# duckdb-faiss-ext/duckdb-faiss-ext

Hardware: AMD Instinct MI355X
Metric: queries/sec, FlatL2 d=128 N=10000000 nq=10000 k=10 (higher is better)
Workload: dtype f32 results (bf16 matrix-pipe coarse filter with a proven bound + exact f32 re-scoring of the candidates); 1 GPU; Flat L2 d=128 N=10000000 nq=10000 k=10; queries_per_call=10000, replicas=1, exchange=none

## Files before the change

duckdb-faiss-ext_amd/csrc/collect_launch.h:

```cpp
#pragma once
#include "common.h"

#include <algorithm>
#include <cmath>
#include <cstddef>
#include <cstdint>

namespace mvs {

struct CandStream {
	unsigned long long *entries = nullptr;
	float *values = nullptr;
	unsigned long long *count = nullptr;
	int64_t cap = 0;
};
struct FailList {
	int *count = nullptr;
	int *queries = nullptr;
};

bool collect_supported(const FlatGeom &g);
void launch_collect_mean(const FlatGeom &g, const float *d_vecs, int64_t nrows, float *d_mu, hipStream_t st);
struct CollectStoreRows {
	int metric = 0;
// ... 12 lines not shown
	const float *vecs = nullptr;
	int64_t row0 = 0, nrows = 0;
	const float *mu = nullptr, *beta = nullptr;
	float sy = 0.f, unit = 0.f;
	signed char *i8 = nullptr;
	int *beta_i = nullptr;
	unsigned *bits = nullptr;
};
void launch_rows_to_i8(const FlatGeom &g, const CollectI8Rows &r, hipStream_t st);
void launch_collect_outlier_threshold(const float *d_norms, int64_t nrows, const float *d_mu, int dp, unsigned *d_max_norm_bits, hipStream_t st);
void launch_collect_append_outliers(const int *d_outl, int n_outliers, int64_t nq, const CandStream &s, const unsigned long long *d_rowmask,
                                    hipStream_t st);
size_t collect_qfrag_bytes(const FlatGeom &g, int64_t nq);
const char *collect_wide_kernel_name(int dp1);
size_t collect_qfrag_bytes_ex(int dp1, int qblock, int64_t nq);
int collect_slot_stride(int kk, int dp1);
int collect_max_k(int d);

struct CollectQueryPrep {
	int metric = 0;
	const float *x = nullptr;
	int64_t nq = 0;
	int d = 0;
	const float *mu = nullptr;
	const unsigned *max_norm_bits = nullptr;
	void *qf = nullptr;
	float *qn = nullptr;
	float *e2 = nullptr;
	FailList fail;
	unsigned *gslot = nullptr;
	int stride = 0;
// ... 11 lines not shown
void launch_collect_rowmask(SelectorDev sel, const int64_t *d_idmap, int64_t n, unsigned long long *d_mask, hipStream_t st);

struct CollectPass {
	FlatGeom g;
	int metric = 0;
	const void *qf = nullptr;
	const unsigned short *rows = nullptr;
	const float *beta = nullptr;
	int64_t n = 0, nq = 0;
	int kf = 0;
	const float *e2 = nullptr;
	unsigned *gslot = nullptr;
	const unsigned long long *rowmask = nullptr;
	float *pbnd = nullptr;
	float i8_unit = 0.f;
	hipStream_t st = nullptr;
};
struct CollectPrepare {
	unsigned long long *stream_cnt = nullptr;
	bool cnt_zeroed = false, slots_ready = false;
	float *seed_stage = nullptr;
};
void launch_collect_prepare(const CollectPass &p, const CollectPrepare &pr);
size_t collect_seed_stage_bytes(int64_t nq);
struct CollectScanInfo {
	int grid = 0, nsplit = 0, lds = 0;
	int64_t items = 0;
};
CollectScanInfo launch_collect_scan(const CollectPass &p, const CandStream &s, bool frozen);
struct CollectBigRanges {
	int ranges = 0;
	int64_t rows = 0;
	float *stage = nullptr;
};
void launch_collect_big_bounds(const CollectPass &p, const CollectBigRanges &r);
void launch_collect_big_bounds_seed(const CollectPass &p, const CollectBigRanges &r);
struct CollectDropHeavy {
	const unsigned long long *stream = nullptr;
	int64_t n = 0, nq = 0;
// ... 249 lines not shown
```

duckdb-faiss-ext_amd/csrc/flat_coarse.hip:

```cpp
#include "flat_collect.h"
#include "collect_launch.h"
#include "index.h"

#include <algorithm>
#include <cstring>

namespace mvs {

void FlatIndex::ensure_h1_rows(hipStream_t st) {
	if (h1_rows == ntotal && vecs_h1)
		return;
	const int dp1 = collect_store_dims(d);
	if (!d_max_norm_bits) {
		MVS_HIP(hipMalloc((void **)&d_max_norm_bits, 64));
		MVS_HIP(hipMemsetAsync(d_max_norm_bits, 0, 64, st));
	}
	if (!mu_h1) {
		MVS_HIP(hipMalloc((void **)&mu_h1, (size_t)std::max(geom.dp, 1024) * sizeof(float)));
		const int64_t nm = std::min<int64_t>(ntotal, (int64_t)1 << 20);
		launch_collect_mean(geom, vecs, nm, mu_h1, st);
		const unsigned inf_bits = 0x7f800000u;
		MVS_HIP(hipMemcpyAsync(d_max_norm_bits + CL_NORM_TAU, &inf_bits, sizeof inf_bits, hipMemcpyHostToDevice, st));
		if (ntotal >= 262144 && outlier_rows) {
			MVS_HIP(hipMalloc((void **)&d_outl, (size_t)(1 + CL_OUTL_CAP) * sizeof(int)));
// ... 178 lines not shown
	return (bytes + 255) & ~(size_t)255;
}
static CandStream collect_stream(const CollectWork &w) {
	CandStream s;
	s.entries = w.stream, s.values = w.stream_s, s.count = &w.ctl->count, s.cap = w.cap_entries;
	return s;
}

CollectPlan FlatIndex::collect_plan(const CollectRequest &rq) const {
	CollectPlan pl;
	const int64_t nq = rq.nq;
	const int kk = rq.kk, kf = (rq.kf <= 0 || rq.kf > kk) ? kk : rq.kf;
	pl.kf = kf;
	pl.has_sel = rq.params && rq.params->sel_kind != MVS_SEL_NONE;
	pl.dp1 = collect_store_dims(d);
	pl.stride = collect_slot_stride(kf, pl.dp1);
	pl.wide = pl.dp1 > 128;
	pl.few = !pl.wide && nq <= 128 && pl.stride == 16 && ntotal < ((int64_t)1 << 31);
	pl.bigk = kf > 128;
	pl.bk_seed = pl.bigk && !pl.wide;
	constexpr int bk_per = 8;
	pl.bk_ranges = pl.bigk ? (pl.bk_seed ? (kf + bk_per - 1) / bk_per : (kf + 63) / 64) : 0;
	if (pl.bk_seed) {
		const int nqb = (int)((nq + 511) / 512);
		if (nqb * pl.bk_ranges < 256 && pl.bk_ranges < 64)
			pl.bk_ranges = std::max(pl.bk_ranges, std::min(256 / nqb, 4 * pl.bk_ranges));
	}
	if (pl.bigk) {
		const bool whole = (nq >= 512 && kf >= 512) || (double)nq * kf * 16.0 > (double)((int64_t)1 << 28);
		const int64_t want = whole ? ntotal : std::max<int64_t>(ntotal / 4, (int64_t)pl.bk_ranges * (pl.bk_seed ? 2048 : 16384));
		pl.bk_rows = std::min<int64_t>(std::max<int64_t>(want / pl.bk_ranges, pl.bk_seed ? 1024 : 4096), ntotal / pl.bk_ranges) / 64 * 64;
		if (ntotal / std::max(pl.bk_ranges, 1) < 192 || pl.bk_rows < 64) {
			pl.ok = false;
// ... 58 lines not shown
		qp.cursors = collect_cursors((float *)ws_pbnd.p, nq);
		launch_collect_query_prep(qp, st);
	} else {
		ws_pfq.reserve(collect_qfrag_bytes_ex(pl.dp1, collect_wide_qblock(pl.dp1), nq));
		qp.qf = ws_pfq.p;
		launch_collect_pack_queries_ex(qp, pl.dp1, collect_wide_qblock(pl.dp1), st);
		if (metric == METRIC_L2)
			launch_query_norms(rq.d_x, nq, d, (float *)ws_qn.p, st);
		launch_collect_bounds(qp, st);
	}
	w.cap_entries = pl.cap_entries;
	collect_workspaces(pl, nq, w);
	if (pl.wide)
		MVS_HIP(hipMemsetAsync(ws_seg.p, 0, sizeof(CollectCtl) + (size_t)2 * nq * sizeof(int), st));
	if (!pl.wide)
		ws_seed.reserve(collect_seed_stage_bytes(nq));
	CollectPass &p = w.pass;
	p.g = geom, p.metric = metric, p.qf = ws_pfq.p, p.n = ntotal, p.nq = nq, p.kf = pl.kf;
	p.e2 = (const float *)ws_e2.p, p.gslot = (unsigned *)ws_gthr.p, p.st = st;
	p.pbnd = (pl.wide && !pl.bigk) ? nullptr : (float *)ws_pbnd.p;
	if (pl.bigk) {
		CollectBigRanges r;
		r.ranges = pl.bk_ranges, r.rows = pl.bk_rows;
		if (pl.bk_seed) {
			r.stage = (float *)ws_seed.p;
			launch_collect_big_bounds_seed(p, r);
		} else
			launch_collect_big_bounds(p, r);
	} else {
		CollectPrepare pr;
		pr.stream_cnt = &w.ctl->count, pr.cnt_zeroed = true, pr.slots_ready = !pl.wide;
// ... 207 lines not shown
		if (!res.report_cnt)
			MVS_HIP(hipMemcpyAsync(h_cl_hdr, w.ctl, sizeof(CollectCtl), hipMemcpyDeviceToHost, st));
	} else {
		rs.stream = w.stream, rs.sorted = w.sorted, rs.cnt = w.defer ? &w.ctl->count : nullptr;
		rs.ncand = w.defer ? res.deferred_cap : ncand;
		launch_collect_rescore(rs, st);
		res.tie.sorted = w.sorted;
	}
}

CollectResult FlatIndex::collect_candidates(const CollectRequest &rq) {
	CollectResult res;
	hipStream_t st = rq.st;
	CollectWork w;
	ensure_h1_rows(st);
	const CollectPlan pl = collect_plan(rq);
	if (pl.has_sel) {
		SelectorDev sel = selector.upload(rq.params, st);
		ws_rowmask.reserve(collect_rowmask_bytes(ntotal));
		launch_collect_rowmask(sel, rq.d_idmap, ntotal, (unsigned long long *)ws_rowmask.p, st);
		w.pass.rowmask = (const unsigned long long *)ws_rowmask.p;
	}
	if (!pl.ok)
		return res;
	const bool use_i8 = !pl.wide && !pl.few && ensure_i8_rows(st);
	w.pass.i8_unit = use_i8 ? i8_unit : 0.f;
	w.pass.rows = use_i8 ? (const unsigned short *)vecs_i8 : vecs_h1;
	w.pass.beta = use_i8 ? (const float *)beta_i8 : beta_h1;
	w.defer = rq.defer_count && !pl.bigk;
	collect_prepare(rq, pl, w);
	if (!collect_scan(rq, pl, w, res))
		return res;
	if (pl.fb && collect_finish_bucketed(rq, pl, w, res)) {
		res.emitted = true;
	} else {
		if (pl.fb && rq.flags)
			MVS_HIP(hipMemsetAsync(rq.flags->count, 0, sizeof(int), st));
		collect_finish_sorted(rq, pl, w, res);
	}
	set_kinfo(pl.wide ? collect_wide_kernel_name(pl.dp1) : "flat_bf16_collect_kernel", 2.0 * (double)rq.nq * (double)ntotal * d,
	          (double)ntotal * (pl.dp1 * 2.0 + 4.0) + (double)rq.nq * d * 4.0 + (double)rq.nq * rq.kk * 12.0, w.grid, pl.few ? 64 : 256, w.lds,
	          w.nsplit);
	res.ok = true;
// ... 229 lines not shown
```

duckdb-faiss-ext_amd/csrc/flat_collect.h:

```cpp
#pragma once

#include <cstddef>
#include <cstdint>
#include <vector>

#ifdef __HIPCC__
#define MVS_PLAN_HD __host__ __device__
#else
#define MVS_PLAN_HD
#endif

namespace mvs {

constexpr int CL_SCHED_LEVELS = 12;
constexpr int CL_BODY_MIN_ROWS = 7680;
constexpr int CL_BODY_MAX_RANGES = 384;
constexpr int CL_TAPER_ROUNDS = 2;
constexpr int CL_TAPER_FLOOR_ROWS = 512;
constexpr unsigned CL_ITEM_NONE = 0xffffffffu;

struct CollectSched {
	int nlev, nranges;
	int first[CL_SCHED_LEVELS];
	int rows[CL_SCHED_LEVELS];
// ... 43 lines not shown
inline std::vector<int64_t> collect_plan_ranges(int64_t n_rows, int64_t stage_rows, int64_t nqb, int64_t slots) {
	const CollectSched s = collect_plan_levels(n_rows, stage_rows, nqb, slots);
	std::vector<int64_t> b;
	for (int l = 0; l < s.nlev; ++l) {
		const int end = l + 1 < s.nlev ? s.first[l + 1] : s.nranges;
		for (int r = s.first[l]; r < end; ++r)
			b.push_back(s.begin[l] + (int64_t)(r - s.first[l]) * s.rows[l]);
	}
	b.push_back(n_rows > 0 ? n_rows : 0);
	return b;
}
MVS_PLAN_HD inline int64_t collect_queue_items(int nranges, int x, int64_t nqb) {
	return nranges > x ? (int64_t)((nranges - x + 7) >> 3) * nqb : 0;
}

constexpr int CL_QCOLS = 16;
constexpr unsigned CL_QLAYOUT_FULL_N = 0x924u;
MVS_PLAN_HD inline int collect_qblock_cols(int nq, int qb) {
	const int live = nq - qb * 32 * CL_QCOLS;
	return live >= 32 * CL_QCOLS ? CL_QCOLS : (live <= 0 ? 0 : (live + 31) >> 5);
}
MVS_PLAN_HD inline unsigned collect_qblock_wave(int nq, int qb, int sub_tiles, int wave) {
	const int T = collect_qblock_cols(nq, qb);
	const int own = T >> 2, r = T & 3, spare = 4 - own;
	if (T == CL_QCOLS || sub_tiles != 4 || (r == 3 && spare == 1))
		return (unsigned)(4 * wave) * 0x1111u + 0x3210u + (CL_QLAYOUT_FULL_N << 16);
	const int pair = wave >> 1, half = wave & 1;
	unsigned cols = 0xFFFFu;
	unsigned n = 0x249u * (unsigned)own;
#define MVS_QB_PUT(slot, col) cols = (cols & ~(15u << (4 * (slot)))) | ((unsigned)(col) << (4 * (slot)))
// ... 155 lines not shown
```

duckdb-faiss-ext_amd/csrc/flat_collect.hip:

```cpp
#include "flat_collect.h"
#include "collect_launch.h"

#include <algorithm>
#include <climits>
#include <cmath>
#include <cstring>
#include <type_traits>

#include <rocprim/device/device_radix_sort.hpp>
#include <rocprim/device/device_segmented_radix_sort.hpp>

namespace mvs {

__global__ __launch_bounds__(256) void collect_colsum_kernel(const float *__restrict__ src, long long nrows, int dp,
                                                            int interleaved, float *__restrict__ sum) {
	const int g8 = dp / 8, rl = threadIdx.x / g8, c8 = threadIdx.x % g8, nrl = 256 / g8;
	float acc[8] = {0.f, 0.f, 0.f, 0.f, 0.f, 0.f, 0.f, 0.f};
	const long long r0 = (long long)blockIdx.x * 1024;
	__shared__ float red[256 * 8];
	const bool idle = rl >= nrl;
	for (long long r = r0 + rl; !idle && r < r0 + 1024 && r < nrows; r += nrl) {
		const float4 s0 = *(const float4 *)(src + (size_t)r * dp + c8 * 8);
		const float4 s1 = *(const float4 *)(src + (size_t)r * dp + c8 * 8 + 4);
		float v[8];
// ... 577 lines not shown
	constexpr int PITCH = I8 ? DP : DP * 2;
	constexpr int C = PITCH / 16;
	constexpr int TILE_BYTES = CL_BN * PITCH;
	constexpr int SUB = cl_sub(I8);
	constexpr int STAGE_ROWS = SUB * CL_BN;
	constexpr int STAGE_BYTES = SUB * TILE_BYTES;
	constexpr int NDMA = STAGE_BYTES / 1024;
	constexpr int DMA_PER_WAVE = NDMA / 4;
	constexpr int QCAP = cl_qcap(I8);
	static_assert(C == (I8 ? 8 : 16) && KB == (I8 ? 2 : 4) && NDMA % 4 == 0 && STAGE_ROWS % 64 == 0, "d = 128 geometry");
	typedef typename std::conditional<I8, i32x4n, bf16x8>::type frag_t;
	typedef typename std::conditional<I8, i32x4n, f32x4acc>::type acc_t;
	typedef typename std::conditional<I8, i32x2n, f32x2n>::type bnd_t;
	typedef typename std::conditional<I8, int, float>::type val_t;
	const float unit = a.i8_unit;

	extern __shared__ __attribute__((aligned(16))) float smem[];
	char *tbuf = (char *)smem;
	float *nbuf = (float *)(tbuf + 2 * STAGE_BYTES);
	unsigned long long *qbuf = (unsigned long long *)(nbuf + 2 * STAGE_ROWS);
	float *cqtab = (float *)(qbuf + QCAP);
	unsigned *qctl = (unsigned *)(cqtab + CL_QBLOCK);
	float *qval = (float *)(qctl + 16);
	float *cqstage = qval + QCAP;

	const int tid = threadIdx.x, lane = tid & 63;
	const int wave = __builtin_amdgcn_readfirstlane(tid >> 6);
	const int hq = lane >> 4, c = lane & 15;
	unsigned *const cursors = a.cursors;
	auto take = [&]() -> unsigned {
// ... 5 lines not shown
			if ((dead >> x) & 1u)
				continue;
			const unsigned cnt = (unsigned)collect_queue_items(sc.nranges, x, a.nqb);
			const unsigned j = cnt ? __hip_atomic_fetch_add(cursors + x * CL_CURSOR_STRIDE, 1u, __ATOMIC_RELAXED, __HIP_MEMORY_SCOPE_AGENT) : 0u;
			if (cnt && j < cnt)
				got = (j << 3) | (unsigned)x;
			else
				dead |= 1u << x;
		}
		qctl[10] = dead;
		return got;
	};
	struct Item {
		long long rb, re;
		int qb, rng;
	};
	auto decode = [&](unsigned w) {
		Item it;
		const unsigned x = w & 7u, j = w >> 3;
		const unsigned rr = j / (unsigned)a.nqb;
		it.qb = __builtin_amdgcn_readfirstlane((int)(j - rr * (unsigned)a.nqb));
		it.rng = __builtin_amdgcn_readfirstlane((int)(rr * 8u + x));
		typedef __attribute__((address_space(4))) const CollectSched csched;
		unsigned long long scp = (unsigned long long)(uintptr_t)((__attribute__((address_space(4))) const char *)__builtin_amdgcn_kernarg_segment_ptr() +
		                                                         offsetof(CollectLaunch, sc));
		asm volatile("" : "+s"(scp));
		csched *p = (csched *)(uintptr_t)scp;
		const int nlev = p->nlev;
		int lev = 0;
#pragma unroll 1
		for (int l = 1; l < nlev && it.rng >= p->first[l]; ++l)
			lev = l;
		const int f = p->first[lev], rw = p->rows[lev];
		const long long bg = p->begin[lev];
		it.rb = a.row_first + bg + (long long)(it.rng - f) * rw;
		it.re = it.rb + rw < a.n ? it.rb + rw : a.n;
		return it;
	};
	if (tid == 0) {
		qctl[7] = 0u;
		qctl[10] = 0u;
		qctl[8] = take();
	}
	__syncthreads();
	unsigned curw = (unsigned)__builtin_amdgcn_readfirstlane((int)qctl[8]);
	int hw = 0;
	long long r_begin = 0, r_end = 0;
	int qb = -1;
	unsigned lay = 0u;
	frag_t bq[8][KB];

// ... 181 lines not shown
#pragma unroll
			for (int kb = 0; kb < KB; ++kb)
				bq[cb][kb] = qsrc[(qblk16 * KB + kb) * 64 + lane];
		}
	}
	if (!staged) {
#pragma unroll
		for (int i = 0; i < DMA_PER_WAVE; ++i)
			dma_issue(r_begin, par, i);
		dma_norms(r_begin, par);
		if (use_tab && newq)
			dma_bounds(qb);
		__syncthreads();
		tab_cvt();
	}
	const int duty_phase = it.rng * 13 + 5;
	for (int u = 0; u < ntiles; ++u) {
		const bool pull = u + 2 == ntiles || ntiles < 2;
		bool hand = false;
		long long nx_rb = 0;
		int nx_qb = qb;
		if (u == ntiles - 1 && ntiles >= 2) {
			const unsigned nxtw = (unsigned)__builtin_amdgcn_readfirstlane((int)qctl[8 + (hw ^ 1)]);
			hand = nxtw != CL_ITEM_NONE;
			if (hand) {
				const Item nx = decode(nxtw);
				nx_rb = nx.rb, nx_qb = nx.qb;
			}
		}
		const int period = u < 4 ? 1 : (u < 32 ? 8 : (u < 256 ? 32 : 128));
		const bool full = !frozen && (use_tab ? ((u + duty_phase) & duty_mask) == 0 : (u % period) == 0);
		if (use_tab && hand && nx_qb != qb)
			dma_bounds(nx_qb);
		else if (use_tab && !full && u > 0 && (u & ((1 << tab_shift) - 1)) == 0)
			dma_bounds(qb);
		if (full) {
			publish();
			int qo = qb * CL_QBLOCK + 32 * collect_qblock_slot_col(lay, hq);
			MVS_OPAQUE_VGPR(qo);
			f32x2n v = {0.f, 0.f};
#pragma unroll 1
			for (int i = 0; i < 2; ++i) {
				const int q = qo + 16 * i + c;
				const int qc = q < a.nq ? q : 0;
				const float e2v = __builtin_nontemporal_load(a.e2 + qc);
				constexpr int SUBN = NC > 32 ? 32 : NC, NSUB = NC / SUBN;
				const int rank = NSUB == 1 ? a.nclass - 1 : (a.nclass + NSUB - 1) / NSUB - 1;
				unsigned kth = 0u;
#pragma unroll 1
// ... 428 lines not shown
			MVS_CL_GO(true, true, 16)
		else
			MVS_CL_GO(false, true, 16)
	} else if (metric == METRIC_L2) {
		MVS_CL_GO(true, false, 16)
	} else {
		MVS_CL_GO(false, false, 16)
	}
#undef MVS_CL_GO
	MVS_HIP(hipGetLastError());
	if (grid_out)
		*grid_out = grid;
}


template <bool IS_L2, bool SEL, bool I8 = false>
__global__ __launch_bounds__(256, 2) void flat_bf16_seed_kernel(const CollectArgs a) {
	constexpr int KB = I8 ? 2 : 4, PITCH = I8 ? 128 : 256, C = PITCH / 16;
	constexpr int TILE_BYTES = CL_BN * PITCH, STAGE_BYTES = CL_SUB * TILE_BYTES;
	constexpr int DMA_PER_WAVE = STAGE_BYTES / 4096;
	typedef typename std::conditional<I8, i32x4n, bf16x8>::type frag_t;
	typedef typename std::conditional<I8, i32x4n, f32x4acc>::type acc_t;
	typedef typename std::conditional<I8, int, float>::type val_t;
	const val_t lowest = I8 ? (val_t)INT_MIN : (val_t)-INFINITY;
	extern __shared__ __attribute__((aligned(16))) float smem[];
	float *nbuf = (float *)((char *)smem + 2 * STAGE_BYTES);
	const int tid = threadIdx.x, lane = tid & 63;
	const int wave = __builtin_amdgcn_readfirstlane(tid >> 6);
	const int hq = lane >> 4, c = lane & 15;
	const int split = blockIdx.x / a.nqb, qb = blockIdx.x % a.nqb;
	const long long r_begin = a.row_first + (long long)split * a.split_rows;
	long long r_end = r_begin + (a.split_len > 0 ? a.split_len : a.split_rows);
// ... 19 lines not shown
	}
	auto dma_block = [&](int u) {
#pragma unroll
		for (int i = 0; i < DMA_PER_WAVE; ++i) {
			const char *base = (const char *)a.yb + (size_t)(r_begin + (long long)u * (CL_SUB * CL_BN)) * PITCH + (size_t)i * 4096;
			__builtin_amdgcn_global_load_lds((glb_f32c *)(base + dma_off),
			                                 (lds_f32c *)(smem + ((u & 1) * STAGE_BYTES + (i * 4 + wave) * 1024) / 4), 16, 0, 0);
		}
		const float *nb = a.yn + (r_begin + (long long)u * (CL_SUB * CL_BN));
		__builtin_amdgcn_global_load_lds((glb_f32c *)(nb + lane), (lds_f32c *)(smem + (2 * STAGE_BYTES) / 4 + (u & 1) * 64), 4, 0, 0);
	};
	if (ntiles > 0)
		dma_block(0);
	__syncthreads();
	const unsigned rbase = (unsigned)(c * PITCH) | (unsigned)(((hq ^ c) & (C - 1)) * 16);
	acc_t cm[8];
#pragma unroll
	for (int cb = 0; cb < 8; ++cb)
		cm[cb] = acc_t {lowest, lowest, lowest, lowest};
	for (int u = 0; u < ntiles; ++u) {
#pragma unroll 1
		for (int sub = 0; sub < CL_SUB; ++sub) {
			frag_t A[KB][2];
			acc_t Y[2];
			{
				const unsigned nb_lds = (unsigned)(uintptr_t)((lds_f32c *)(nbuf + (u & 1) * 64 + sub * CL_BN + 4 * hq));
				asm volatile("ds_read_b128 %0, %2\n\tds_read_b128 %1, %2 offset:64" : "=&v"(Y[0]), "=&v"(Y[1]) : "v"(nb_lds) : "memory");
				const unsigned ab = (unsigned)(uintptr_t)((lds_f32c *)(smem + ((u & 1) * STAGE_BYTES + sub * TILE_BYTES) / 4)) + rbase;
#pragma unroll
				for (int kb = 0; kb < KB; ++kb) {
					asm volatile("ds_read_b128 %0, %1" : "=v"(A[kb][0]) : "v"(ab ^ (unsigned)(kb * 64)) : "memory");
					if (I8)
						asm volatile("ds_read_b128 %0, %1 offset:2048" : "=v"(A[kb][1]) : "v"(ab ^ (unsigned)(kb * 64)) : "memory");
					else
// ... 11 lines not shown
			if constexpr (I8)
				asm volatile("s_waitcnt lgkmcnt(0)" : "+v"(Y[0]), "+v"(Y[1]), "+v"(A[0][0]), "+v"(A[0][1]), "+v"(A[1][0]), "+v"(A[1][1]));
			else
				asm volatile("s_waitcnt lgkmcnt(0)"
				             : "+v"(Y[0]), "+v"(Y[1]), "+v"(A[0][0]), "+v"(A[0][1]), "+v"(A[1][0]), "+v"(A[1][1]), "+v"(A[2][0]), "+v"(A[2][1]),
				               "+v"(A[3][0]), "+v"(A[3][1]));
			acc_t acc[2][2];
			auto fold = [&](int rb, int t) {
#pragma unroll
				for (int i = 0; i < 2; ++i)
#pragma unroll
					for (int r = 0; r < 4; ++r) {
						val_t v = acc[rb][i][r];
						if (SEL)
							v = ((rowbits >> (16 * rb + 4 * hq + r)) & 1u) ? v : lowest;
						if constexpr (I8)
							cm[2 * t + i][r] = cm[2 * t + i][r] > v ? cm[2 * t + i][r] : v;
						else
							cm[2 * t + i][r] = __builtin_fmaxf(cm[2 * t + i][r], v);
					}
			};
#pragma unroll
			for (int t = 0; t < 4; ++t) {
#pragma unroll
				for (int rb = 0; rb < 2; ++rb) {
#pragma unroll
					for (int kb = 0; kb < KB; ++kb) {
#pragma unroll
						for (int i = 0; i < 2; ++i) {
							if constexpr (I8)
								acc[rb][i] = __builtin_amdgcn_mfma_i32_16x16x64_i8(A[kb][rb], bq[2 * t + i][kb], kb == 0 ? Y[rb] : acc[rb][i], 0, 0, 0);
							else if (kb == 0)
								acc[rb][i] = __builtin_amdgcn_mfma_f32_16x16x32_bf16(A[kb][rb], bq[2 * t + i][kb], Y[rb], 0, 0, 0);
							else
// ... 1 lines not shown
						}
						if (kb == 1 && (t > 0 || rb > 0))
							fold(rb ^ 1, rb == 0 ? t - 1 : t);
						__builtin_amdgcn_sched_barrier(0);
					}
				}
			}
			fold(1, 3);
		}
		__syncthreads();
	}
	asm volatile("s_waitcnt vmcnt(0)" ::: "memory");
#pragma unroll
	for (int cb = 0; cb < 8; ++cb) {
		const int q = qw + 16 * cb + c;
		f32x4acc m;
#pragma unroll
		for (int r = 0; r < 4; ++r)
			m[r] = I8 ? (cm[cb][r] == lowest ? -INFINITY : (float)cm[cb][r] * a.i8_unit) : (float)cm[cb][r];
		if (q < a.nq)
			*(f32x4acc *)(a.seed_stage + ((size_t)split * (size_t)a.nq + (size_t)q) * 16 + 4 * hq) = m;
	}
}
__global__ void collect_seed_reduce_kernel(const float *__restrict__ stage, int nsplit, long long nq, unsigned *__restrict__ gslot) {
	const long long i = (long long)blockIdx.x * blockDim.x + threadIdx.x;
	if (i >= nq * 4)
		return;
	f32x4acc m = {-INFINITY, -INFINITY, -INFINITY, -INFINITY};
	for (int s = 0; s < nsplit; ++s) {
		const f32x4acc v = *(const f32x4acc *)(stage + ((size_t)s * (size_t)nq * 16) + (size_t)i * 4);
#pragma unroll
		for (int r = 0; r < 4; ++r)
			m[r] = __builtin_fmaxf(m[r], v[r]);
	}
#pragma unroll
	for (int r = 0; r < 4; ++r)
		if (m[r] > -INFINITY) {
			const unsigned k = skey(m[r]);
			unsigned *p = gslot + (size_t)i * 4 + r;
			*p = k < *p ? k : *p;
		}
}
static void launch_collect_seed(int metric, CollectArgs a, int64_t rows, int64_t nq, hipStream_t st) {
	const int nqb = (int)((nq + CL_QBLOCK - 1) / CL_QBLOCK);
	const int64_t nblocks = rows / (CL_SUB * CL_BN);
	if (nblocks <= 0)
		return;
	const int64_t nsplit = std::max<int64_t>(1, std::min<int64_t>(std::max<int64_t>(8, 512 / nqb), nblocks / 8));
	a.row_first = 0;
	a.split_rows = (nblocks + nsplit - 1) / nsplit * (CL_SUB * CL_BN);
	a.n = nblocks * (CL_SUB * CL_BN);
	a.nqb = nqb;
	a.nsplit = (int)((nblocks * (CL_SUB * CL_BN) + a.split_rows - 1) / a.split_rows);
	const int grid = nqb * a.nsplit;
	const size_t lds = (size_t)2 * CL_SUB * CL_BN * 256 + 2 * 64 * 4 + 64;
#define MVS_SEED(L2, SL)                                                                                           \
	{                                                                                                              \
		auto kern = a.i8_unit > 0.f ? flat_bf16_seed_kernel<L2, SL, true> : flat_bf16_seed_kernel<L2, SL>;         \
		ensure_dynamic_lds((const void *)kern, lds);                                                               \
		hipLaunchKernelGGL(kern, dim3(grid), dim3(256), lds, st, a);                                               \
	}
	if (metric == METRIC_L2 && a.rowmask)
		MVS_SEED(true, true)
	else if (metric == METRIC_L2)
		MVS_SEED(true, false)
	else if (a.rowmask)
		MVS_SEED(false, true)
	else
		MVS_SEED(false, false)
#undef MVS_SEED
	hipLaunchKernelGGL(collect_seed_reduce_kernel, dim3((unsigned)((nq * 4 + 255) / 256)), dim3(256), 0, st, (const float *)a.seed_stage, a.nsplit,
		                   (long long)nq, a.gslot);
	MVS_HIP(hipGetLastError());
}
size_t collect_seed_stage_bytes(int64_t nq) {
	return (size_t)64 * (size_t)nq * 16 * sizeof(float);
}

int collect_slot_stride(int kk, int dp1) {
	if (dp1 == 128 && kk > 28)
		return 128;
	if (dp1 > 128 && kk > 32 && collect_wide_max_classes(dp1) >= 128)
		return 128;
	return kk > 16 ? 32 : 16;
}
int collect_max_k(int d) {
	const int dp1 = collect_store_dims(d);
	if (dp1 == 0)
		return 0;
	if (dp1 == 128)
		return 128;
	return collect_wide_max_classes(dp1);
}

template <int NC>
__global__ void collect_final_thr_kernel(const unsigned *__restrict__ gslot, const float *__restrict__ e2, int nclass, long long nq,
                                         float *__restrict__ thr) {
	const long long q = (long long)blockIdx.x * blockDim.x + threadIdx.x;
	if (q >= nq)
// ... 161 lines not shown
			launch_collect_wide_range(dp1, p.metric, false, a, r0, r1, std::max<int64_t>(8, std::min<int64_t>(64, 1024 / nqbw)), nq, st, nullptr, nullptr);
		} else {
			a.pbnd = p.pbnd;
			launch_collect_range<false>(p.g, p.metric, a, r0, r1, nq, st, nullptr, nullptr, nullptr);
		}
	}
	const long long total = dp1 > 128 ? (long long)nq : (long long)nqb * CL_QBLOCK;
	hipLaunchKernelGGL(collect_bound_table_multi_kernel, dim3((unsigned)((total + 127) / 128)), dim3(128), 0, st, (const unsigned *)p.gslot,
	                   (long long)nq * 128, nranges, p.e2, kfp, (int)nq, total, p.pbnd, dp1 > 128 ? 1 : 0, cl_sub(p.i8_unit > 0.f));
	MVS_HIP(hipGetLastError());
}

void launch_collect_final_thr(const CollectPass &p, float *d_thr) {
	if (p.nq <= 0)
		return;
	const int stride = collect_slot_stride(p.kf, collect_store_dims(p.g.d));
	const dim3 grid((unsigned)((p.nq + 63) / 64));
	if (stride == 128)
		hipLaunchKernelGGL(collect_final_thr_kernel<128>, grid, dim3(64), 0, p.st, (const unsigned *)p.gslot, p.e2, p.kf, (long long)p.nq, d_thr);
	else if (stride == 32)
		hipLaunchKernelGGL(collect_final_thr_kernel<32>, grid, dim3(64), 0, p.st, (const unsigned *)p.gslot, p.e2, p.kf, (long long)p.nq, d_thr);
	else
		hipLaunchKernelGGL(collect_final_thr_kernel<16>, grid, dim3(64), 0, p.st, (const unsigned *)p.gslot, p.e2, p.kf, (long long)p.nq, d_thr);
	MVS_HIP(hipGetLastError());
}

__global__ void collect_report_kernel(const unsigned long long *__restrict__ hdr, const int *__restrict__ fail_cnt,
                                      const unsigned *__restrict__ maxnorm, int *__restrict__ h_flags,
                                      unsigned long long *__restrict__ h_hdr, int with_cnt) {
	const int t = threadIdx.x;
	if (h_hdr && hdr && t < 32)
// ... 6 lines not shown
			h_flags[10] = (int)(unsigned)c;
			h_flags[11] = (int)(unsigned)(c >> 32);
		}
	}
}
void launch_collect_report(const CollectReportSrc &r, hipStream_t st) {
	hipLaunchKernelGGL(collect_report_kernel, dim3(1), dim3(64), 0, st, (const unsigned long long *)r.hdr, r.fail_cnt, r.maxnorm, r.h_flags,
	                   (unsigned long long *)r.h_hdr, r.with_cnt ? 1 : 0);
	MVS_HIP(hipGetLastError());
}

void launch_collect_prepare(const CollectPass &p, const CollectPrepare &pr) {
	const int64_t n = p.n, nq = p.nq;
	const int kk = p.kf, metric = p.metric;
	hipStream_t st = p.st;
	const int stride = collect_slot_stride(kk, collect_store_dims(p.g.d));
	const long long gtotal = (long long)nq * stride;
	if (!pr.slots_ready)
		hipLaunchKernelGGL(init_gslot_kernel, dim3((unsigned)((gtotal + 255) / 256)), dim3(256), 0, st, p.gslot, gtotal, stride, stride,
		                   0 );
	if (!pr.cnt_zeroed)
		MVS_HIP(hipMemsetAsync(pr.stream_cnt, 0, 16, st));
	CollectArgs a = collect_base_args(p, p.gslot, stride, kk);
	a.pbnd = p.pbnd;
	const int dp1 = collect_store_dims(p.g.d);
	if (dp1 == 128 && stride == 16) {
		constexpr int64_t seed_reg_rows = 32768;
		const int64_t rows = std::min<int64_t>(seed_reg_rows, n / 8) / 64 * 64;
		if (rows >= 1024) {
			a.seed_stage = pr.seed_stage;
			launch_collect_seed(metric, a, rows, nq, st);
		}
		return;
	}
	constexpr int64_t seed_rows = 16384, seed_split = 32;
	const int64_t kscale = std::max(1, kk / 16);
	const int64_t seed = std::min<int64_t>(n, kscale * std::min<int64_t>(seed_rows, std::max<int64_t>(2048, n / 256)));
	if (seed > 0 && seed < n) {
		if (dp1 > 128)
			launch_collect_wide_range(dp1, metric, false, a, 0, seed, seed_split, nq, st, nullptr, nullptr);
		else
			launch_collect_range<false>(p.g, metric, a, 0, seed, nq, st, nullptr, nullptr, nullptr);
	}
}

CollectScanInfo launch_collect_scan(const CollectPass &p, const CandStream &out, bool frozen) {
	const int64_t n = p.n, nq = p.nq;
	const int dp1 = collect_store_dims(p.g.d);
	CollectArgs a = collect_base_args(p, p.gslot, frozen ? 16 : collect_slot_stride(p.kf, dp1), frozen ? 16 : p.kf);
	a.stream = out.entries;
	a.stream_s = out.values;
	a.stream_cnt = out.count;
	a.stream_cap = out.cap;
	a.flags = frozen ? CL_FROZEN : 0;
	a.pbnd = p.pbnd;
	CollectScanInfo info;
	const int qblock = dp1 > 128 ? collect_wide_qblock(dp1) : CL_QBLOCK;
	const int nqb = (int)((nq + qblock - 1) / qblock);
	if (dp1 > 128) {
		const int64_t slots = collect_wide_slots(dp1);
		const int64_t max_split = std::max<int64_t>(1, n / 7680);
		int64_t nsplit = 1;
		double best = -1;
		for (int64_t s = 8; s <= std::min<int64_t>(max_split, 512); s += 8) {
// ... 521 lines not shown
```

duckdb-faiss-ext_amd/csrc/index.h:

```cpp
#pragma once
#include "common.h"

#include "../../include/mi355_faiss.h"

#include <functional>
#include <memory>
#include <mutex>
#include <string>
#include <utility>
#include <vector>

namespace mvs {

struct DevBuf {
	void *p = nullptr;
	size_t cap = 0;
	void reserve(size_t bytes);
	void release();
	~DevBuf() {
		release();
	}
};

struct PinnedRing {
// ... 411 lines not shown
	bool cl_fbucket_off = false;
	int cl_skip = 0, cl_skip_len = 0;
	int64_t cl_queries_total = 0, cl_candidates_total = 0, cl_overflows = 0, cl_last_candidates = 0, cl_heavy_total = 0;
	int64_t cl_scan_items = 0, cl_scan_ranges = 0;
	int64_t cl_last_rescored = -1, cl_rescored_total = 0, cl_rescored_queries = 0, cl_admitted_in_fb = 0;
	DevBuf ws_e2, ws_stream, ws_sorttmp, ws_seg, ws_rowmask, ws_items1, ws_qcount;
	void ensure_bf16_rows(hipStream_t st);
	void ensure_h1_rows(hipStream_t st);
	signed char *vecs_i8 = nullptr;
	int *beta_i8 = nullptr;
	unsigned *d_i8_bits = nullptr;
	int64_t i8_cap = 0, i8_rows = 0;
	float i8_sy = 0.f, i8_unit = 0.f;
	int i8_state = 0;
	bool cl_i8 = true;
	bool ensure_i8_rows(hipStream_t st);
	void drop_i8();
	int *d_outl = nullptr;
	int h1_outliers = 0;
	int64_t outl_total = 0;
	bool outlier_rows = true;
	bool coarse_topk(int64_t nq, const float *d_x, int64_t np, float *d_D, int64_t *d_I, hipStream_t st, bool need_matrix = true);
	DevBuf ws_cb16;
	int64_t cb16_queries = 0;
	size_t cb16_stats_off = 0;
	int64_t cb16_last_nq = 0;
	size_t cb16_ccount_off = 0;
	const float *coarse_matrix() const {
		return (const float *)ws_q.p;
	}
// ... 231 lines not shown
```

duckdb-faiss-ext_amd/csrc/index.hip:

```cpp
#include "coded_lists.h"
#include "flat_collect.h"
#include "collect_launch.h"
#include "index.h"

#include <atomic>
#include <condition_variable>
#include <map>
#include <mutex>
#include <optional>
#include <thread>

#include <algorithm>
#include <dlfcn.h>
#include <chrono>
#include <cstdarg>
#include <cstdlib>
#include <cstring>

namespace mvs {

static thread_local std::string g_last_error;

void set_last_error(const char *what) {
	g_last_error = what;
// ... 2185 lines not shown
		p = static_cast<IDMapIndex *>(p)->sub;
	if (name && strncmp(name, "pretransform_", 13) != 0)
		if (IndexBase *inner = pretransform_sub_of(p))
			p = inner;
	if (!name || !value)
		throw_faiss("mvs_index_get_stat", __FILE__, "null argument");
	if (!strcmp(name, "flat_outlier_rows")) {
		if (p->kind != MVS_KIND_FLAT)
			throw_faiss("mvs_index_get_stat", __FILE__, "%s: not a Flat index", name);
		*value = static_cast<FlatIndex *>(p)->outl_total;
	} else if (!strcmp(name, "cl_store_i8")) {
		if (p->kind != MVS_KIND_FLAT)
			throw_faiss("mvs_index_get_stat", __FILE__, "%s: not a Flat index", name);
		const auto *f = static_cast<FlatIndex *>(p);
		*value = f->cl_i8 && f->i8_state == 1 ? 1 : 0;
	} else if (!strcmp(name, "cl_scan_items") || !strcmp(name, "cl_scan_ranges")) {
		if (p->kind != MVS_KIND_FLAT)
			throw_faiss("mvs_index_get_stat", __FILE__, "%s: not a Flat index", name);
		const auto *f = static_cast<FlatIndex *>(p);
		*value = !strcmp(name, "cl_scan_items") ? f->cl_scan_items : f->cl_scan_ranges;
	} else if (!strcmp(name, "coarse_bf16_queries") || !strcmp(name, "coarse_bf16_exhaustive") || !strcmp(name, "coarse_bf16_candidates")) {
		IndexBase *qz = ivf_quantizer_of(p);
		if (!qz || qz->kind != MVS_KIND_FLAT)
			throw_faiss("mvs_index_get_stat", __FILE__, "%s: not an IVF index with a Flat quantizer", name);
		auto *f = static_cast<FlatIndex *>(qz);
		if (!strcmp(name, "coarse_bf16_queries")) {
			*value = f->cb16_queries;
		} else if (!strcmp(name, "coarse_bf16_candidates")) {
			int64_t sum = 0;
			if (f->ws_cb16.p && f->cb16_last_nq > 0) {
// ... 284 lines not shown
	for (const Key &e : keys) {
		if (strcmp(key, e.name))
			continue;
		tune_.*(e.field) = e.flag ? v != 0 : (int)v;
		return true;
	}
	return false;
}
bool FlatIndex::set_option(const char *key, int64_t v) {
	if (set_tuning(key, v))
		return true;
	if (!strcmp(key, "cl_i8")) {
		cl_i8 = v != 0;
		return true;
	}
	if (!strcmp(key, "outlier_rows")) {
		outlier_rows = v != 0;
		return true;
	}
	if (!strcmp(key, "lazy_adds")) {
		flush_adds();
		lazy_adds = v != 0;
		return true;
	}
	if (!strcmp(key, "metric_arg_bits")) {
		const uint32_t b = (uint32_t)v;
		memcpy(&metric_arg, &b, 4);
		return true;
	}
	if (!strcmp(key, "force_staged")) {
// ... 75 lines not shown
```

Baseline: 1.055 million queries/s.

## Pace collect-scan threshold upkeep by rows seen; add optional 32 row classes for int8

On the int8 collect path, the scan kernel now sets how often it recomputes and publishes thresholds, and how often it refetches bounds, from how many rows earlier ranges have already covered. It starts at a floor period and doubles it as more of the table has been seen, so late ranges spend less time on upkeep once thresholds have settled. Separately, the seed kernel, seed reduce and slot-stride logic gain a 32-class variant for the int8 store; it is chosen via a `cl_classes` option or automatically when k is at least 15, and a new stat reports the class count. Less frequent upkeep can leave thresholds looser for longer, so the scan may emit more candidates, and 32 classes use more registers in the seed kernel.

```diff
diff --git a/duckdb-faiss-ext_amd/csrc/collect_launch.h b/duckdb-faiss-ext_amd/csrc/collect_launch.h
--- a/duckdb-faiss-ext_amd/csrc/collect_launch.h
+++ b/duckdb-faiss-ext_amd/csrc/collect_launch.h
@@ -50,7 +50,8 @@
 size_t collect_qfrag_bytes(const FlatGeom &g, int64_t nq);
 const char *collect_wide_kernel_name(int dp1);
 size_t collect_qfrag_bytes_ex(int dp1, int qblock, int64_t nq);
-int collect_slot_stride(int kk, int dp1);
+constexpr int CL_I8_CLASSES32_FROM = 15;
+int collect_slot_stride(int kk, int dp1, bool i8);
 int collect_max_k(int d);
 
 struct CollectQueryPrep {
@@ -92,15 +93,17 @@
 	const unsigned long long *rowmask = nullptr;
 	float *pbnd = nullptr;
 	float i8_unit = 0.f;
+	int classes = 0;
 	hipStream_t st = nullptr;
 };
+int collect_pass_stride(const CollectPass &p);
 struct CollectPrepare {
 	unsigned long long *stream_cnt = nullptr;
 	bool cnt_zeroed = false, slots_ready = false;
 	float *seed_stage = nullptr;
 };
 void launch_collect_prepare(const CollectPass &p, const CollectPrepare &pr);
-size_t collect_seed_stage_bytes(int64_t nq);
+size_t collect_seed_stage_bytes(int64_t nq, int nc);
 struct CollectScanInfo {
 	int grid = 0, nsplit = 0, lds = 0;
 	int64_t items = 0;
diff --git a/duckdb-faiss-ext_amd/csrc/flat_coarse.hip b/duckdb-faiss-ext_amd/csrc/flat_coarse.hip
--- a/duckdb-faiss-ext_amd/csrc/flat_coarse.hip
+++ b/duckdb-faiss-ext_amd/csrc/flat_coarse.hip
@@ -216,9 +216,9 @@
 	pl.kf = kf;
 	pl.has_sel = rq.params && rq.params->sel_kind != MVS_SEL_NONE;
 	pl.dp1 = collect_store_dims(d);
-	pl.stride = collect_slot_stride(kf, pl.dp1);
+	pl.stride = collect_slot_stride(kf, pl.dp1, false);
 	pl.wide = pl.dp1 > 128;
-	pl.few = !pl.wide && nq <= 128 && pl.stride == 16 && ntotal < ((int64_t)1 << 31);
+	pl.few = !pl.wide && nq <= 128 && kf <= 16 && ntotal < ((int64_t)1 << 31);
 	pl.bigk = kf > 128;
 	pl.bk_seed = pl.bigk && !pl.wide;
 	constexpr int bk_per = 8;
@@ -307,7 +307,7 @@
 	if (pl.wide)
 		MVS_HIP(hipMemsetAsync(ws_seg.p, 0, sizeof(CollectCtl) + (size_t)2 * nq * sizeof(int), st));
 	if (!pl.wide)
-		ws_seed.reserve(collect_seed_stage_bytes(nq));
+		ws_seed.reserve(collect_seed_stage_bytes(nq, pl.stride));
 	CollectPass &p = w.pass;
 	p.g = geom, p.metric = metric, p.qf = ws_pfq.p, p.n = ntotal, p.nq = nq, p.kf = pl.kf;
 	p.e2 = (const float *)ws_e2.p, p.gslot = (unsigned *)ws_gthr.p, p.st = st;
@@ -545,7 +545,7 @@
 	hipStream_t st = rq.st;
 	CollectWork w;
 	ensure_h1_rows(st);
-	const CollectPlan pl = collect_plan(rq);
+	CollectPlan pl = collect_plan(rq);
 	if (pl.has_sel) {
 		SelectorDev sel = selector.upload(rq.params, st);
 		ws_rowmask.reserve(collect_rowmask_bytes(ntotal));
@@ -558,6 +558,10 @@
 	w.pass.i8_unit = use_i8 ? i8_unit : 0.f;
 	w.pass.rows = use_i8 ? (const unsigned short *)vecs_i8 : vecs_h1;
 	w.pass.beta = use_i8 ? (const float *)beta_i8 : beta_h1;
+	w.pass.g = geom, w.pass.kf = pl.kf, w.pass.classes = cl_classes;
+	if (!pl.bigk && !pl.few)
+		pl.stride = collect_pass_stride(w.pass);
+	cl_row_classes = pl.bigk ? 0 : pl.stride;
 	w.defer = rq.defer_count && !pl.bigk;
 	collect_prepare(rq, pl, w);
 	if (!collect_scan(rq, pl, w, res))
diff --git a/duckdb-faiss-ext_amd/csrc/flat_collect.h b/duckdb-faiss-ext_amd/csrc/flat_collect.h
--- a/duckdb-faiss-ext_amd/csrc/flat_collect.h
+++ b/duckdb-faiss-ext_amd/csrc/flat_collect.h
@@ -81,6 +81,40 @@
 	return nranges > x ? (int64_t)((nranges - x + 7) >> 3) * nqb : 0;
 }
 
+constexpr int CL_UPKEEP_FLOOR_ROWS = 8192;
+constexpr int CL_UPKEEP_CEIL_ROWS = 131072;
+constexpr int CL_UPKEEP_SHARE = 4;
+constexpr int CL_UPKEEP_FETCH_DIV = 32;
+constexpr int CL_UPKEEP_FETCH_FLOOR_ROWS = 256;
+struct CollectUpkeep {
+	int derive, fetch;
+};
+MVS_PLAN_HD inline CollectUpkeep collect_upkeep_periods(long long seen_rows, int stage_rows) {
+	CollectUpkeep up;
+	const int ceil_st = CL_UPKEEP_CEIL_ROWS / stage_rows;
+	up.derive = CL_UPKEEP_FLOOR_ROWS / stage_rows;
+	while (up.derive < ceil_st && 2ll * up.derive * stage_rows * CL_UPKEEP_SHARE <= seen_rows)
+		up.derive *= 2;
+	up.fetch = CL_UPKEEP_FETCH_FLOOR_ROWS / stage_rows;
+	while (up.fetch * 2 * CL_UPKEEP_FETCH_DIV <= up.derive)
+		up.fetch *= 2;
+	return up;
+}
+template <class S> MVS_PLAN_HD inline long long collect_range_begin(const S *p, int r) {
+	const int nlev = p->nlev;
+	int lev = 0;
+	for (int l = 1; l < nlev && r >= p->first[l]; ++l)
+		lev = l;
+	return p->begin[lev] + (long long)(r - p->first[lev]) * p->rows[lev];
+}
+template <class S> MVS_PLAN_HD inline long long collect_seen_rows(const S *p, int rng, int nqb, int slots) {
+	const int at_work = (slots + nqb - 1) / nqb;
+	return rng > at_work ? collect_range_begin(p, rng - at_work) : 0;
+}
+MVS_PLAN_HD inline bool collect_upkeep_due(int u, int rng, int derive) {
+	return ((u + rng * 13 + 5) & (derive - 1)) == 0;
+}
+
 constexpr int CL_QCOLS = 16;
 constexpr unsigned CL_QLAYOUT_FULL_N = 0x924u;
 MVS_PLAN_HD inline int collect_qblock_cols(int nq, int qb) {
diff --git a/duckdb-faiss-ext_amd/csrc/flat_collect.hip b/duckdb-faiss-ext_amd/csrc/flat_collect.hip
--- a/duckdb-faiss-ext_amd/csrc/flat_collect.hip
+++ b/duckdb-faiss-ext_amd/csrc/flat_collect.hip
@@ -615,6 +615,7 @@
 	typedef typename std::conditional<I8, i32x2n, f32x2n>::type bnd_t;
 	typedef typename std::conditional<I8, int, float>::type val_t;
 	const float unit = a.i8_unit;
+	constexpr bool PACED = I8 && COLLECT && NC <= 32;
 
 	extern __shared__ __attribute__((aligned(16))) float smem[];
 	char *tbuf = (char *)smem;
@@ -650,6 +651,7 @@
 	struct Item {
 		long long rb, re;
 		int qb, rng;
+		long long seen;
 	};
 	auto decode = [&](unsigned w) {
 		Item it;
@@ -671,6 +673,7 @@
 		const long long bg = p->begin[lev];
 		it.rb = a.row_first + bg + (long long)(it.rng - f) * rw;
 		it.re = it.rb + rw < a.n ? it.rb + rw : a.n;
+		it.seen = PACED ? collect_seen_rows(p, it.rng, a.nqb, (int)gridDim.x) : 0;
 		return it;
 	};
 	if (tid == 0) {
@@ -882,7 +885,13 @@
 		__syncthreads();
 		tab_cvt();
 	}
-	const int duty_phase = it.rng * 13 + 5;
+	int derive = duty_mask + 1, fetch = 1 << tab_shift;
+	bool refetch = false;
+	if (PACED && use_tab && !frozen) {
+		const CollectUpkeep up = collect_upkeep_periods(it.seen, STAGE_ROWS);
+		derive = up.derive, fetch = up.fetch;
+		refetch = !newq;
+	}
 	for (int u = 0; u < ntiles; ++u) {
 		const bool pull = u + 2 == ntiles || ntiles < 2;
 		bool hand = false;
@@ -897,10 +906,10 @@
 			}
 		}
 		const int period = u < 4 ? 1 : (u < 32 ? 8 : (u < 256 ? 32 : 128));
-		const bool full = !frozen && (use_tab ? ((u + duty_phase) & duty_mask) == 0 : (u % period) == 0);
+		const bool full = !frozen && (use_tab ? collect_upkeep_due(u, it.rng, derive) : (u % period) == 0);
 		if (use_tab && hand && nx_qb != qb)
 			dma_bounds(nx_qb);
-		else if (use_tab && !full && u > 0 && (u & ((1 << tab_shift) - 1)) == 0)
+		else if (use_tab && !full && (u > 0 || refetch) && (u & (fetch - 1)) == 0)
 			dma_bounds(qb);
 		if (full) {
 			publish();
@@ -1359,8 +1368,10 @@
 }
 
 
-template <bool IS_L2, bool SEL, bool I8 = false>
+template <bool IS_L2, bool SEL, bool I8 = false, int NC = 16>
 __global__ __launch_bounds__(256, 2) void flat_bf16_seed_kernel(const CollectArgs a) {
+	static_assert(NC == 16 || (NC == 32 && I8), "32 classes: the int8 store only");
+	constexpr int NRB = NC / 16;
 	constexpr int KB = I8 ? 2 : 4, PITCH = I8 ? 128 : 256, C = PITCH / 16;
 	constexpr int TILE_BYTES = CL_BN * PITCH, STAGE_BYTES = CL_SUB * TILE_BYTES;
 	constexpr int DMA_PER_WAVE = STAGE_BYTES / 4096;
@@ -1410,10 +1421,12 @@
 		dma_block(0);
 	__syncthreads();
 	const unsigned rbase = (unsigned)(c * PITCH) | (unsigned)(((hq ^ c) & (C - 1)) * 16);
-	acc_t cm[8];
+	acc_t cm[8][NRB];
 #pragma unroll
 	for (int cb = 0; cb < 8; ++cb)
-		cm[cb] = acc_t {lowest, lowest, lowest, lowest};
+#pragma unroll
+		for (int b = 0; b < NRB; ++b)
+			cm[cb][b] = acc_t {lowest, lowest, lowest, lowest};
 	for (int u = 0; u < ntiles; ++u) {
 #pragma unroll 1
 		for (int sub = 0; sub < CL_SUB; ++sub) {
@@ -1455,10 +1468,11 @@
 						val_t v = acc[rb][i][r];
 						if (SEL)
 							v = ((rowbits >> (16 * rb + 4 * hq + r)) & 1u) ? v : lowest;
+						acc_t &m = cm[2 * t + i][NRB == 2 ? rb : 0];
 						if constexpr (I8)
-							cm[2 * t + i][r] = cm[2 * t + i][r] > v ? cm[2 * t + i][r] : v;
+							m[r] = m[r] > v ? m[r] : v;
 						else
-							cm[2 * t + i][r] = __builtin_fmaxf(cm[2 * t + i][r], v);
+							m[r] = __builtin_fmaxf(m[r], v);
 					}
 			};
 #pragma unroll
@@ -1490,21 +1504,24 @@
 #pragma unroll
 	for (int cb = 0; cb < 8; ++cb) {
 		const int q = qw + 16 * cb + c;
-		f32x4acc m;
-#pragma unroll
-		for (int r = 0; r < 4; ++r)
-			m[r] = I8 ? (cm[cb][r] == lowest ? -INFINITY : (float)cm[cb][r] * a.i8_unit) : (float)cm[cb][r];
-		if (q < a.nq)
-			*(f32x4acc *)(a.seed_stage + ((size_t)split * (size_t)a.nq + (size_t)q) * 16 + 4 * hq) = m;
-	}
-}
-__global__ void collect_seed_reduce_kernel(const float *__restrict__ stage, int nsplit, long long nq, unsigned *__restrict__ gslot) {
+#pragma unroll
+		for (int b = 0; b < NRB; ++b) {
+			f32x4acc m;
+#pragma unroll
+			for (int r = 0; r < 4; ++r)
+				m[r] = I8 ? (cm[cb][b][r] == lowest ? -INFINITY : (float)cm[cb][b][r] * a.i8_unit) : (float)cm[cb][b][r];
+			if (q < a.nq)
+				*(f32x4acc *)(a.seed_stage + ((size_t)split * (size_t)a.nq + (size_t)q) * NC + 16 * b + 4 * hq) = m;
+		}
+	}
+}
+__global__ void collect_seed_reduce_kernel(const float *__restrict__ stage, int nsplit, long long quads, unsigned *__restrict__ gslot) {
 	const long long i = (long long)blockIdx.x * blockDim.x + threadIdx.x;
-	if (i >= nq * 4)
+	if (i >= quads)
 		return;
 	f32x4acc m = {-INFINITY, -INFINITY, -INFINITY, -INFINITY};
 	for (int s = 0; s < nsplit; ++s) {
-		const f32x4acc v = *(const f32x4acc *)(stage + ((size_t)s * (size_t)nq * 16) + (size_t)i * 4);
+		const f32x4acc v = *(const f32x4acc *)(stage + ((size_t)s * (size_t)quads + (size_t)i) * 4);
 #pragma unroll
 		for (int r = 0; r < 4; ++r)
 			m[r] = __builtin_fmaxf(m[r], v[r]);
@@ -1522,7 +1539,7 @@
 	const int64_t nblocks = rows / (CL_SUB * CL_BN);
 	if (nblocks <= 0)
 		return;
-	const int64_t nsplit = std::max<int64_t>(1, std::min<int64_t>(std::max<int64_t>(8, 512 / nqb), nblocks / 8));
+	const int64_t nsplit = std::max<int64_t>(1, std::min<int64_t>(std::min<int64_t>(64, std::max<int64_t>(8, 512 / nqb)), nblocks / 8));
 	a.row_first = 0;
 	a.split_rows = (nblocks + nsplit - 1) / nsplit * (CL_SUB * CL_BN);
 	a.n = nblocks * (CL_SUB * CL_BN);
@@ -1530,9 +1547,12 @@
 	a.nsplit = (int)((nblocks * (CL_SUB * CL_BN) + a.split_rows - 1) / a.split_rows);
 	const int grid = nqb * a.nsplit;
 	const size_t lds = (size_t)2 * CL_SUB * CL_BN * 256 + 2 * 64 * 4 + 64;
+	if (a.slot_stride == 32 && !(a.i8_unit > 0.f))
+		throw Error("flat_bf16_seed_kernel: 32 row classes on the bf16 store");
 #define MVS_SEED(L2, SL)                                                                                           \
 	{                                                                                                              \
-		auto kern = a.i8_unit > 0.f ? flat_bf16_seed_kernel<L2, SL, true> : flat_bf16_seed_kernel<L2, SL>;         \
+		auto kern = a.i8_unit > 0.f ? (a.slot_stride == 32 ? flat_bf16_seed_kernel<L2, SL, true, 32> : flat_bf16_seed_kernel<L2, SL, true>) \
+		                            : flat_bf16_seed_kernel<L2, SL>;                                               \
 		ensure_dynamic_lds((const void *)kern, lds);                                                               \
 		hipLaunchKernelGGL(kern, dim3(grid), dim3(256), lds, st, a);                                               \
 	}
@@ -1545,20 +1565,28 @@
 	else
 		MVS_SEED(false, false)
 #undef MVS_SEED
-	hipLaunchKernelGGL(collect_seed_reduce_kernel, dim3((unsigned)((nq * 4 + 255) / 256)), dim3(256), 0, st, (const float *)a.seed_stage, a.nsplit,
-		                   (long long)nq, a.gslot);
+	const long long quads = (long long)nq * (a.slot_stride / 4);
+	hipLaunchKernelGGL(collect_seed_reduce_kernel, dim3((unsigned)((quads + 255) / 256)), dim3(256), 0, st, (const float *)a.seed_stage, a.nsplit,
+		                   quads, a.gslot);
 	MVS_HIP(hipGetLastError());
 }
-size_t collect_seed_stage_bytes(int64_t nq) {
-	return (size_t)64 * (size_t)nq * 16 * sizeof(float);
-}
-
-int collect_slot_stride(int kk, int dp1) {
+size_t collect_seed_stage_bytes(int64_t nq, int nc) {
+	return (size_t)64 * (size_t)nq * (size_t)nc * sizeof(float);
+}
+
+int collect_slot_stride(int kk, int dp1, bool i8) {
 	if (dp1 == 128 && kk > 28)
 		return 128;
 	if (dp1 > 128 && kk > 32 && collect_wide_max_classes(dp1) >= 128)
 		return 128;
-	return kk > 16 ? 32 : 16;
+	return kk > 16 || (i8 && dp1 == 128 && kk >= CL_I8_CLASSES32_FROM) ? 32 : 16;
+}
+int collect_pass_stride(const CollectPass &p) {
+	const int dp1 = collect_store_dims(p.g.d);
+	const bool i8 = dp1 == 128 && p.i8_unit > 0.f;
+	if (i8 && p.kf <= 16 && (p.classes == 16 || p.classes == 32))
+		return p.classes;
+	return collect_slot_stride(p.kf, dp1, i8);
 }
 int collect_max_k(int d) {
 	const int dp1 = collect_store_dims(d);
@@ -1750,7 +1778,7 @@
 void launch_collect_final_thr(const CollectPass &p, float *d_thr) {
 	if (p.nq <= 0)
 		return;
-	const int stride = collect_slot_stride(p.kf, collect_store_dims(p.g.d));
+	const int stride = collect_pass_stride(p);
 	const dim3 grid((unsigned)((p.nq + 63) / 64));
 	if (stride == 128)
 		hipLaunchKernelGGL(collect_final_thr_kernel<128>, grid, dim3(64), 0, p.st, (const unsigned *)p.gslot, p.e2, p.kf, (long long)p.nq, d_thr);
@@ -1787,7 +1815,7 @@
 	const int64_t n = p.n, nq = p.nq;
 	const int kk = p.kf, metric = p.metric;
 	hipStream_t st = p.st;
-	const int stride = collect_slot_stride(kk, collect_store_dims(p.g.d));
+	const int stride = collect_pass_stride(p);
 	const long long gtotal = (long long)nq * stride;
 	if (!pr.slots_ready)
 		hipLaunchKernelGGL(init_gslot_kernel, dim3((unsigned)((gtotal + 255) / 256)), dim3(256), 0, st, p.gslot, gtotal, stride, stride,
@@ -1797,7 +1825,7 @@
 	CollectArgs a = collect_base_args(p, p.gslot, stride, kk);
 	a.pbnd = p.pbnd;
 	const int dp1 = collect_store_dims(p.g.d);
-	if (dp1 == 128 && stride == 16) {
+	if (dp1 == 128 && (stride == 16 || (stride == 32 && a.i8_unit > 0.f))) {
 		constexpr int64_t seed_reg_rows = 32768;
 		const int64_t rows = std::min<int64_t>(seed_reg_rows, n / 8) / 64 * 64;
 		if (rows >= 1024) {
@@ -1820,7 +1848,7 @@
 CollectScanInfo launch_collect_scan(const CollectPass &p, const CandStream &out, bool frozen) {
 	const int64_t n = p.n, nq = p.nq;
 	const int dp1 = collect_store_dims(p.g.d);
-	CollectArgs a = collect_base_args(p, p.gslot, frozen ? 16 : collect_slot_stride(p.kf, dp1), frozen ? 16 : p.kf);
+	CollectArgs a = collect_base_args(p, p.gslot, frozen ? 16 : collect_pass_stride(p), frozen ? 16 : p.kf);
 	a.stream = out.entries;
 	a.stream_s = out.values;
 	a.stream_cnt = out.count;
diff --git a/duckdb-faiss-ext_amd/csrc/index.h b/duckdb-faiss-ext_amd/csrc/index.h
--- a/duckdb-faiss-ext_amd/csrc/index.h
+++ b/duckdb-faiss-ext_amd/csrc/index.h
@@ -449,6 +449,8 @@
 	float i8_sy = 0.f, i8_unit = 0.f;
 	int i8_state = 0;
 	bool cl_i8 = true;
+	int cl_classes = 0;
+	int cl_row_classes = 0;
 	bool ensure_i8_rows(hipStream_t st);
 	void drop_i8();
 	int *d_outl = nullptr;
diff --git a/duckdb-faiss-ext_amd/csrc/index.hip b/duckdb-faiss-ext_amd/csrc/index.hip
--- a/duckdb-faiss-ext_amd/csrc/index.hip
+++ b/duckdb-faiss-ext_amd/csrc/index.hip
@@ -2223,6 +2223,10 @@
 			throw_faiss("mvs_index_get_stat", __FILE__, "%s: not a Flat index", name);
 		const auto *f = static_cast<FlatIndex *>(p);
 		*value = f->cl_i8 && f->i8_state == 1 ? 1 : 0;
+	} else if (!strcmp(name, "cl_row_classes")) {
+		if (p->kind != MVS_KIND_FLAT)
+			throw_faiss("mvs_index_get_stat", __FILE__, "%s: not a Flat index", name);
+		*value = static_cast<FlatIndex *>(p)->cl_row_classes;
 	} else if (!strcmp(name, "cl_scan_items") || !strcmp(name, "cl_scan_ranges")) {
 		if (p->kind != MVS_KIND_FLAT)
 			throw_faiss("mvs_index_get_stat", __FILE__, "%s: not a Flat index", name);
@@ -2537,6 +2541,12 @@
 		cl_i8 = v != 0;
 		return true;
 	}
+	if (!strcmp(key, "cl_classes")) {
+		if (v != 0 && v != 16 && v != 32)
+			throw_faiss("set_option", __FILE__, "cl_classes: 0, 16 or 32");
+		cl_classes = (int)v;
+		return true;
+	}
 	if (!strcmp(key, "outlier_rows")) {
 		outlier_rows = v != 0;
 		return true;
```

Measured after the change: 1.092 million queries/s, median of 6. 3.5% higher.
